# GoatWu/AdaLog

Hardware: AMD Instinct MI355X
Metric: calib_images_per_sec (higher is better)
Workload: dtype bf16

## Files before the change

### adalog_amd/_lib.py

```python
import ctypes as C
import os

_HERE = os.path.dirname(os.path.abspath(__file__))
LIB_PATH = os.environ.get("ADALOG_LIB") or os.path.join(_HERE, "csrc", "libadalog_hip.so")

p, i32, i64, f32, f64 = C.c_void_p, C.c_int, C.c_int64, C.c_float, C.c_double

ABI_VERSION = 2

SIGNATURES = {
    "adalog_abi_version": (i32, []),
    "adalog_last_error": (C.c_char_p, []),
    "adalog_last_kernel": (C.c_char_p, []),
    "adalog_uniform_fake_quant_f32": (i32, [p, p, p, i64, p, p, i64, i64, i32, i32, p]),
    "adalog_pack_uniform": (i32, [p, i64, i64, i64, i64, i64, i64, p, p, i64, i64, i64, i64, i64, i32, i32, p, i64, p, i32, p]),
    "adalog_pack_raw_f32": (i32, [p, i64, i64, i64, i64, i64, i64, p, i64, p]),
    "adalog_pack_split3_bf16": (i32, [p, i64, i64, i64, i64, i64, i64, p, i64, p]),
    "adalog_gemm_score": (i32, [i32, p, p, i64, i64, i64, i64, i32, i32, i64, i64, i32, i32, i32, p, i64, i64, i64, i32,
                                p, i64, i64, f32, p, i64, i64, i64, p, i64, i64, i64, p, p, p, i64, p, i64, i64, i64, i32, i32, p]),
    "adalog_gemm_score_layout": (i64, [i32, i32, i32, i32, i32, i32, i32, i32, i64, i64, i32, p, p, p]),
    "adalog_log2_shift": (i32, [p, p, i64, f32, p]),
    "adalog_score_act_fused_ok": (i32, [i32, i64, i32, i64, i32, i32]),
    "adalog_score_act_fused_workspace_bytes": (i64, [i64, i64]),
    "adalog_score_act_fused": (i32, [p, i32, i64, p, p, i64, i32, p, p, p, p, p, i32, i32, p, f32, i32, f32, f64, p, i64, p, p]),
# ... 65 lines not shown
    "adalog_select_hist": (i32, [p, i64, i64, i32, i32, i32, i64, i32, i32, i32, p, p]),
    "adalog_select_pick": (i32, [p, i64, i32, i32, p, i32, p]),
    "adalog_select_quantile_out": (i32, [p, i64, i32, p, i32, p, p]),
    "adalog_select_value_out": (i32, [p, i64, i32, p, p]),
    "adalog_uniform_int_f32": (i32, [p, p, i64, p, p, i32, p]),
    "adalog_permute_heads": (i32, [p, p, i64, i64, i32, i32, i32, i32, p]),
    "adalog_merge_heads": (i32, [p, p, p, p, p, i64, i64, i32, i32, i32, p]),
    "adalog_qkv_quant_chunks": (i32, [i64, i64, i32]),
    "adalog_qkv_split_quant": (i32, [p, p, p, p, i64, i64, i32, i32, p, p, p, p, p]),
    "adalog_qkv_merge_quant_backward": (i32, [p, p, p, p, p, i64, i64, i32, i32, p, p, p, p, p, p, p]),
    "adalog_scaled_softmax": (i32, [p, p, i64, i32, f32, p]),
    "adalog_scaled_softmax_backward": (i32, [p, p, p, i64, i32, f32, p]),
    "adalog_uniform_fq_backward_blocks": (i32, [i64, i64, i64]),
    "adalog_uniform_fq_backward": (i32, [p, p, p, i64, p, p, i64, i64, i32, i32, p, p, p, p]),
    "adalog_uniform_fake_quant_drop_f32": (i32, [p, p, i64, p, p, i64, i64, i32, i32, f32, p, i32, p]),
    "adalog_uniform_fq_backward_drop": (i32, [p, p, p, i64, p, p, i64, i64, i32, i32, p, p, p, f32, p, i32, p]),
    "adalog_log_fake_quant_drop_f32": (i32, [p, p, i64, p, p, i32, p, i32, i32, f32, p, i32, p]),
    "adalog_log_fq_backward_drop": (i32, [p, p, p, i64, p, p, i32, p, i32, p, p, i32, f32, p, i32, p]),
    "adalog_qkv_split_quant_drop": (i32, [p, p, p, p, i64, i64, i32, i32, p, p, p, p, p, p, p, p]),
    "adalog_qkv_merge_quant_backward_drop": (i32, [p, p, p, p, p, i64, i64, i32, i32, p, p, p, p, p, p, p, p, p, p]),
    "adalog_adaround": (i32, [p, p, p, p, i64, i64, p, p, i32, i32, i32, p]),
    "adalog_adaround_t": (i32, [p, p, p, p, i64, i64, p, p, i32, i32, p]),
    "adalog_alpha_step_multi": (i32, [p, p, p, p, p, p, p, p, p, p, i32, f32, p, f32, f32, f32, p, f32, p, f32, p, p, p]),
    "adalog_round_loss": (i32, [p, i64, f32, p, p, p, f32, p, i32, p, p]),
    "adalog_round_loss_multi_workspace": (i64, [p, i32]),
    "adalog_round_loss_multi": (i32, [p, p, p, i32, f32, p, f32, p, p, p, p]),
    "adalog_gemm_win_ok": (i32, [i32, i32, i32, i32, i32, i32, i64]),
    "adalog_gemm_score_gen": (i32, [i32, p, i64, i32, i32, i64, i64, i32, i32, p, i64, i64, p, i32, p, i64, i32, p, i64, i64, f32, p, i64,
                              i64, p, i64, p]),
    "adalog_gemm_score_gen_ok": (i32, [i32, i32, i32, i32, i32, i32, i64, i64]),
    "adalog_gemm_score_avq": (i32, [p, i64, i32, i32, i64, i64, i32, i32, p, i64, i64, p, p, i32, p, i64, i32, p, i64, i64, f32, p, i64, i64,
                              p, i64, p]),
    "adalog_gemm_score_avq_ok": (i32, [i32, i32, i32, i32, i32, i64, i64, i32]),
    "adalog_gemm_mixed_ok": (i32, [i32, i32, i32, i32, i32, i64]),
    "adalog_gemm_mixed_ktrim": (i32, [i32, i32, i32, i32, i32, i64]),
    "adalog_rec_loss": (i32, [p, p, i64, f32, p, p, p]),
    "adalog_rec_loss_backward": (i32, [p, p, i64, f32, p, p, p]),
    "adalog_brecq_init": (i32, []),
    "adalog_adam_multi": (i32, [p, p, p, p, p, i32, f32, p, f32, f32, f32, p, p]),
    "adalog_gemm_f32x3_workspace_bytes": (i64, [i32, i32, i32, i32, i32, i32, i32, i32, i32]),
    "adalog_gemm_f32x3_planes_workspace_bytes": (i64, [i32, i32, i32, i32, i32, i32]),
    "adalog_gemm_f32x3_planes": (i32, [p, i64, p, i64, p, i64, i32, i32, i32, i32, i64, i64, p, f32, p, i32, i32, p, p]),
    "adalog_gemm_f32x3": (i32, [p, i64, i32, p, i64, i32, p, i64, i32, i32, i32, i32, i64, i64, i64, p, f32, p, i32, i32, i32, p, p]),
    "adalog_gemm_f32x3_add": (i32, [p, i64, i32, p, i64, i32, p, i64, i32, i32, i32, i32, i64, i64, i64, p, f32, p, i32, i32, i32, p, p, p]),
    "adalog_gemm_f32x3_g2": (i32, [p, i64, i32, p, i64, i32, p, i64, i32, i32, i32, i32, i64, i64, i64, i32, i64, i64, i64, p, f32, p,
                             i32, i32, i32, p, p]),
    "adalog_shift_fold": (i32, [p, p, p, p, i32, i32, p, p]),
    "adalog_minmax_rows": (i32, [p, i32, i32, i32, p, p, p]),
    "adalog_absminmax_cols": (i32, [p, i64, i32, i32, p, p, p]),
    "adalog_packed_row_words": (i64, [i64, i32]),
    "adalog_pack_codes_f32": (i32, [p, i64, i64, i64, p, p, i32, i32, p, p]),
    "adalog_unpack_codes": (i32, [p, i64, i64, p, p, i32, i32, i32, p, i64, p]),
    "adalog_err_stats_workspace_bytes": (i64, [i64, i64, i64]),
    "adalog_err_stats_f32": (i32, [p, p, i64, i64, i64, p, p, i64, p]),
    "adalog_mean_err_workspace_bytes": (i64, [i64, i64, i64]),
    "adalog_mean_err_f32": (i32, [p, p, i64, i64, i64, p, p, i64, p]),
    "adalog_uniform_code_hist_f32": (i32, [p, i64, p, p, i64, i64, i32, p, p]),
    "adalog_log_code_hist_f32": (i32, [p, i64, p, p, i32, p, i32, p, p]),
    "adalog_gptq_sweep_ok": (i32, [i64, i64]),
    "adalog_gptq_sweep_f32": (i32, [p, i64, i64, i64, p, p, i32, i32, p, i64, p, p, p, p]),
    "adalog_bit_cost_ok": (i32, [i64, i64, i32]),
    "adalog_bit_cost_workspace_bytes": (i64, [i64, i64, i32]),
    "adalog_bit_cost_f32": (i32, [p, i64, i64, i64, p, p, i32, p, i32, p, i64, p, p, i64, p]),
}

class FpcsTail(C.Structure):
# ... 41 lines not shown
```

### adalog_amd/csrc/gemm_score.hip

```cpp
#include "common.h"
#include "fpcs_tail.h"
#include <stdlib.h>

#pragma clang fp contract(fast)

namespace {

#include "gemm_types.inc"
#include "gemm_k_basic.inc"
#include "gemm_k_stream.inc"
#include "gemm_k_slab.inc"
#include "gemm_k_grp.inc"
#include "gemm_finish.inc"

}

static int device_cus() {
    static int n_cu = 0;
    if (!n_cu) {
        int dev = 0; hipDeviceProp_t prop;
        if (hipGetDevice(&dev) == hipSuccess && hipGetDeviceProperties(&prop, dev) == hipSuccess) n_cu = prop.multiProcessorCount;
        if (n_cu <= 0) n_cu = 256;
    }
    return n_cu;
}

static int pick_tm_out(int M, int64_t col_tiles_x_groups) {
    if (const char* e = getenv("ADALOG_GEMM_TM")) { const int v = atoi(e); if (v == 1 || v == 2 || v == 4) return v; }
    const int64_t want = 2 * (int64_t)device_cus();
    const int tms[3] = {4, 2, 1};
    for (int i = 0; i < 3; ++i)
        if ((int64_t)cdiv(M, 64 * tms[i]) * col_tiles_x_groups >= want) return tms[i];
    return 1;
}

static int pick_tm(int M, bool scoring) {
    if (const char* e = getenv("ADALOG_GEMM_TM")) {
        const int v = atoi(e);
        if (v == 1 || v == 2 || (v == 4 && !scoring)) return v;
    }
    double best = 0.0;
    int tms[3] = {scoring ? 2 : 4, 2, 1};
    double util[3];
    for (int i = 0; i < 3; ++i) {
        const int bm = 64 * tms[i];
// ... 603 lines not shown
extern "C" int adalog_gemm_score_avq(const void* A, int64_t sAg, int M, int N, int64_t Kp, int64_t k_valid, int G, int gmod,
                                     const float* x, int64_t ldx, int64_t sg, const float* q, const uint32_t* lut, int n_bits,
                                     const float* ref, int64_t sRg, int P, const float* sa, int64_t sa_c, int64_t sa_g, float sa_mul,
                                     const float* sb, int64_t sb_c, int64_t sb_g, float* partial, int64_t partial_elems,
                                     void* stream) {
    ADALOG_ARG_CHECK(A && x && q && lut && ref && sa && sb && partial, "gemm_score_avq: null pointer");
    ADALOG_ARG_CHECK(avq_ok(M, N, G, gmod, P, k_valid, Kp, n_bits), "gemm_score_avq: shape not taken (adalog_gemm_score_avq_ok)");
    ADALOG_ARG_CHECK((((uintptr_t)A) & 15) == 0 && (((uintptr_t)partial) & 7) == 0, "gemm_score_avq: operand / accumulator alignment");
    const Layout L = layout_of(M, N * P, 1, G, gmod, P, 1, true, k_valid * 2, Kp * 2, true, 1);
    ADALOG_ARG_CHECK(partial_elems >= L.elems, "gemm_score_avq: partial buffer too small");
    GemmArgs p{};
    p.A = (const uint8_t*)A; p.sAg = sAg * 2; p.M = M; p.N = N * P; p.Kb = Kp * 2; p.Kvb = k_valid * 2; p.C = 1; p.G = G; p.gmod = gmod;
    p.ref = ref; p.ldr = 1; p.sRg = sRg; p.ref_cs = M; p.ref_div = P;
    p.sa = sa; p.sa_c = sa_c; p.sa_g = sa_g; p.sa_mul = sa_mul; p.sb = sb; p.sb_c = sb_c; p.sb_g = sb_g;
    p.wg_acc = (double*)partial; p.partial = partial;
    p.gen_x = x; p.gen_ldx = ldx; p.gen_sg = sg; p.gen_K = (int)k_valid; p.gen_q = q; p.gen_lut = lut; p.gen_nb = 1 << n_bits;
    wave_chunks(p, N, L.wgs, G, cdiv(N, AVQ_ROWS));
    const int nks = k_valid <= 64 ? 4 : 13;
    const size_t lut_b = (((size_t)(p.gen_nb + 1) * P + 3) & ~(size_t)3) * 4;
    const size_t rows_b = (size_t)4 * ((size_t)AVQ_ROWS * (nks * 16 + 64) + 4 * 64 * 2) * 4;
    const size_t acc_b = (size_t)gmod * 256 * 8;
    const size_t shm = lut_b + rows_b > acc_b ? lut_b + rows_b : acc_b;
    hipStream_t st = (hipStream_t)stream;
    const unsigned wgs = (unsigned)L.wgs;
    const int e = nks == 13 ? (M > 32 ? adalog_launch<k_gemm_avq<4, 13, 2>>("k_gemm_avq<13,bf16>", 80 * 1024, wgs, 256, shm, st, p)
                                      : adalog_launch<k_gemm_avq<4, 13, 1>>("k_gemm_avq<13,bf16>", 80 * 1024, wgs, 256, shm, st, p))
                            : (M > 32 ? adalog_launch<k_gemm_avq<4, 4, 2>>("k_gemm_avq<4,bf16>", 80 * 1024, wgs, 256, shm, st, p)
                                      : adalog_launch<k_gemm_avq<4, 4, 1>>("k_gemm_avq<4,bf16>", 80 * 1024, wgs, 256, shm, st, p));
    if (e) return e;
    ADALOG_LAUNCH_CHECK("adalog_gemm_score_avq");
    return 0;
}

extern "C" int adalog_gemm_score_gen_ok(int dtype, int M, int N, int G, int gmod, int ref_div, int64_t k_valid, int64_t Kp) {
    if (!(dtype == 0 || dtype == 3) || k_valid < 16 || k_valid > 64 || k_valid % 16 || ref_div < 1 || N % ref_div != 0 || G % gmod) return 0;
    const MmCall c = shape_call(dtype, M, N, G, gmod, ref_div, k_valid, Kp, 1);
    const Route r = route_of(c, call_layout(c, true));
    return (r == R_WIN || r == R_GRPW) ? 1 : 0;
}

static Layout gen_layout(int dtype, int M, int64_t T, int K, int64_t Kp, int P) {
    Layout L{};
    if (!(dtype == 0 || dtype == 3) || !(P == 64 || P == 128 || P == 256) || T < 1 || T * P >= ((int64_t)1 << 31) || K < 16 || K % 16 != 0 ||
        Kp < K) return L;
    return layout_of(M, (int)(T * P), 1, 1, 1, P, 1, true, (int64_t)K, Kp, true, dtype, true);
}

extern "C" int adalog_score_act_gen_ok(int dtype, int M, int64_t T, int K, int64_t Kp, int P) {
    static const int use_gen = getenv("ADALOG_SLAB_GEN") ? atoi(getenv("ADALOG_SLAB_GEN")) : 1;
    if (!use_gen || Kp % BK3 != 0) return 0;
    const Layout L = gen_layout(dtype, M, T, K, Kp, P);
    return (L.slab && L.acc) ? 1 : 0;
}

extern "C" int adalog_score_act_gen_wgs(int dtype, int M, int64_t T, int K, int64_t Kp, int P) {
    const Layout L = gen_layout(dtype, M, T, K, Kp, P);
    return (L.slab && L.acc) ? L.wgs : -1;
}

extern "C" int64_t adalog_score_act_gen_workspace_bytes(int dtype, int M, int64_t T, int K, int64_t Kp, int P) {
    const Layout L = gen_layout(dtype, M, T, K, Kp, P);
    if (!(L.slab && L.acc)) return -1;
    return L.elems * (int64_t)sizeof(float) + ((int64_t)M * 4 + 15) / 16 * 16;
}

extern "C" int adalog_score_act_gen(int dtype, const void* Wp, int M, int64_t Kp, const float* x, int64_t T, int K, int64_t ldx,
// ... 180 lines not shown
```

### adalog_amd/ops.py

```python
from __future__ import annotations

import ctypes
import math
import os
from typing import Optional, Tuple

import torch

from . import _lib, _torch_ops

I8, BF16, F32, FP8 = 0, 1, 2, 3
BF16_FP8 = 4
GEMM_EVENTS = None
_ESZ = {I8: 1, BF16: 2, F32: 4, FP8: 1}
_TORCH_DT = {I8: torch.int8, BF16: torch.bfloat16, F32: torch.float32, FP8: torch.float8_e4m3fn}


def _stream():
    return torch.cuda.current_stream().cuda_stream


def _top(name, *args):
    try:
        return getattr(torch.ops.adalog, name)(*args)
# ... 608 lines not shown


def gemm_score_avq_ok(M: int, N: int, G: int, gmod: int, P: int, k_valid: int, Kp: int, n_bits: int) -> bool:
    return bool(_lib.load().adalog_gemm_score_avq_ok(int(M), int(N), int(G), int(gmod), int(P), int(k_valid), int(Kp), int(n_bits)))


def gemm_score_avq(A, src3, q_all, lut, n_bits: int, M: int, N: int, P: int, G: int, gmod: int, ref, sa: Strided, sb: Strided,
                   norm: float, sa_mul: float = 1.0):
    lib = _lib.load()
    sa, sb = sa.checked(), sb.checked()
    src3, q_all, ref = _f32c(src3, "src"), _f32c(q_all, "q"), _f32c(ref, "ref")
    Gs, Ns, K = src3.shape
    Kp = A.shape[-1]
    assert (Gs, Ns) == (G, N) and A.shape[-2] == M and A.is_contiguous() and A.dtype == torch.bfloat16
    assert lut.dtype == torch.int32 and lut.is_contiguous() and lut.shape == ((1 << n_bits) + 1, P)
    assert ref.shape[-1] == M and ref.shape[-2] == N
    sAg = 0 if A.shape[1] == 1 and G > 1 else A.stride(1)
    sRg = 0 if G == 1 else M * N
    n_part, MT, Npad, mode = _layout(M, N * P, 1, G, gmod, P, 1, BF16, Kp, K, True)
    partial = torch.empty((n_part + 1) // 2, dtype=torch.float64, device=A.device).view(torch.float32)
    if GEMM_EVENTS is not None:
        ev0, ev1 = torch.cuda.Event(enable_timing=True), torch.cuda.Event(enable_timing=True)
        ev0.record()
    rc = lib.adalog_gemm_score_avq(A.data_ptr(), sAg, M, N, Kp, K, G, gmod, src3.data_ptr(), K, N * K, q_all.data_ptr(), lut.data_ptr(),
                                   int(n_bits), ref.data_ptr(), sRg, P, sa.t.data_ptr(), sa.c, sa.g, float(sa_mul), sb.t.data_ptr(),
                                   sb.c, sb.g, partial.data_ptr(), n_part, _stream())
    if GEMM_EVENTS is not None:
        ev1.record()
        GEMM_EVENTS.append((BF16, M, N, K, P, G, ev0, ev1, lib.adalog_last_kernel().decode()))
    _lib.check(rc, "adalog_gemm_score_avq")
    return PendingScores(partial, MT, Npad if mode != 1 else N, Npad, P, G, gmod, False, False, mode, norm, N).finish()


def gemm_out(dtype: int, A, B, M: int, N: int, G: int, gmod: int, sa: Strided, sb: Strided, bias: Optional[Strided],
             sa_mul: float = 1.0, addend=None, heads_last: int = 0):
    lib = _lib.load()
    sa, sb = sa.checked(), sb.checked()
    bias = None if bias is None else bias.checked()
    Kp = A.shape[-1]
    assert B.shape[-1] == Kp and A.dtype == _TORCH_DT[dtype] and B.dtype == _TORCH_DT[dtype]
    sAg = 0 if A.shape[1] == 1 and G > 1 else A.stride(1)
    sBg = 0 if B.shape[1] == 1 and G > 1 else B.stride(1)
    if addend is not None or heads_last:
        assert dtype in (I8, BF16) and sa.c == 0 and sb.c == 0 and (bias is None or bias.c == 0)
        H = int(heads_last)
        if H:
            assert G % H == 0 and addend is None
            out = torch.empty((G // H, M, H, N), dtype=torch.float32, device=A.device)
            ldo, sOg, gi, sOo = H * N, N, H, M * H * N
        else:
            addend = _f32c(addend, "addend")
            assert addend.numel() == G * M * N
            out = torch.empty((G, M, N), dtype=torch.float32, device=A.device)
            ldo, sOg, gi, sOo = N, M * N, 0, 0
        rc = lib.adalog_gemm_out_ex(dtype, A.data_ptr(), B.data_ptr(), sAg, sBg, M, N, Kp, G, gmod, sa.t.data_ptr(), sa.g, float(sa_mul),
                                    sb.t.data_ptr(), sb.g, sb.n, None if bias is None else bias.t.data_ptr(),
                                    0 if bias is None else bias.g, 0 if bias is None else bias.n, _ptr(addend), out.data_ptr(),
                                    ldo, sOg, gi, sOo, _stream())
        _lib.check(rc, "adalog_gemm_out_ex")
        return out
    out = torch.empty((G, M, N), dtype=torch.float32, device=A.device)
    rc = lib.adalog_gemm_score(dtype, A.data_ptr(), B.data_ptr(), 0, sAg, 0, sBg, M, N, Kp, 0, 1, G, gmod, None, 0, 0, 1, 1,
                               sa.t.data_ptr(), sa.c, sa.g, float(sa_mul), sb.t.data_ptr(), sb.c, sb.g, sb.n,
                               None if bias is None else bias.t.data_ptr(),
                               0 if bias is None else bias.c, 0 if bias is None else bias.g,
                               0 if bias is None else bias.n, None, None,
# ... 1278 lines not shown
```

### adalog_amd/quant_layers/matmul.py

```python
import os

import torch
import torch.nn as nn

from .. import backend, search, train_mm
from ..ops import BF16, BF16_FP8, FP8, I8, Strided, pad_k
from ..ops import mixed_k_align as ops_mixed_k_align
from ..quantizers.logarithm import AdaLogQuantizer
from ..quantizers.uniform import UniformQuantizer

MAX_PACK_BYTES = int(os.environ.get('ADALOG_MAX_PACK_GIB', '8')) << 30
GEN_MM = os.environ.get('ADALOG_GEN_MM', 'all')
GEN_AVQ = os.environ.get('ADALOG_GEN_AVQ', '1') != '0'
MIXED_B_SEARCH = os.environ.get('ADALOG_MIXED_B', '1') != '0'
AV_KTRIM = os.environ.get('ADALOG_AV_KTRIM', '1') != '0'


class MinMaxQuantMatMul(nn.Module):
    def __init__(self, A_bit=8, B_bit=8, mode="raw"):
        super().__init__()
        self.mode = mode
        self.A_quantizer = UniformQuantizer(n_bits=A_bit, symmetric=True, channel_wise=False)
        self.B_quantizer = UniformQuantizer(n_bits=B_bit, symmetric=True, channel_wise=False)
        self.raw_input = None
        self.raw_out = None
        self.tmp_input = None
        self.tmp_out = None
        self.calibrated = False

    def forward(self, A, B, a_pre=False, b_pre=False):
        if self.mode == 'raw':
            return A @ B
        if self.mode == "quant_forward":
            return self.quant_forward(A, B, a_pre, b_pre)
        raise NotImplementedError

    def quant_input_A(self, x):
        return self.A_quantizer(x)

    def quant_input_B(self, x):
        return self.B_quantizer(x)

    def quant_forward(self, A, B, a_pre=False, b_pre=False):
        assert self.calibrated, f"Module should be calibrated before run quant_forward for {self}"
        a_sim = A if a_pre else self.quant_input_A(A)
        b_sim = B if b_pre else self.quant_input_B(B)
        if a_sim.requires_grad or b_sim.requires_grad:
            return train_mm.matmul(a_sim, b_sim, heads_last=getattr(self, 'out_heads_last', False))
# ... 90 lines not shown

    def _kalign(self, dt=None):
        G, S, K, Sp = self._dims()
        if self.eq_n not in (64, 128, 256):
            return 128
        if dt in (I8, FP8) and K <= 32 and self._cand_chunk(G * max(S, Sp) * 32) >= self.eq_n:
            be, H = backend.get(), self._heads()
            if be.gemm_win_ok(dt, Sp, S, G, H, self.eq_n, K) and be.gemm_win_ok(dt, S, Sp, G, H, self.eq_n, K):
                return 32
        esz = 1 if dt in (I8, FP8) else 2
        whole = self._cand_chunk(G * max(S, Sp) * pad_k(K, BF16 if esz == 2 else I8, 64) * esz) >= self.eq_n
        return 64 if whole else 128

    def _mixed_kalign(self):
        be = backend.get()
        G, S, K, Sp = self._dims()
        kp = 0
        if AV_KTRIM and K > 64 and hasattr(be, "gemm_mixed_ktrim"):
            kp = be.gemm_mixed_ktrim(S, Sp, G, self._heads(), self.eq_n, K)
        return ops_mixed_k_align(K, kp)

    def _pack_fixed(self, which, dt=I8):
        be = backend.get()
        H = self._heads()
        A, B = self.raw_input
        al = self._kalign(dt)
        if which == "A":
            s, z = self._q_params(self.A_quantizer)
            return be.pack_uniform(self._a3(A), s, z, 1, 0, H, 1 if H > 1 else 0, 0, self.A_quantizer.n_bits, dt, k_align=al)
        s, z = self._q_params(self.B_quantizer)
        return be.pack_uniform(self._bt3_packable(B), s, z, 1, 0, H, 1 if H > 1 else 0, 0, self.B_quantizer.n_bits, dt,
                               k_align=al)

    def _score(self, which, fixed, scale, zp, dt=I8, fixed_sa=None, sa_mul=1.0, defer=False):
        be = backend.get()
        H = self._heads()
        G, S, K, Sp = self._dims()
        A, B = self.raw_input
        P = scale.shape[0]
        src = self._a3(A) if which == "A" else self._bt3_packable(B)
        bits = self.A_quantizer.n_bits if which == "A" else self.B_quantizer.n_bits
        rows = S if which == "A" else Sp
        mixed = dt == BF16_FP8
        cdt = FP8 if mixed else dt
        esz = 2 if dt == BF16 else 1
        al = ops_mixed_k_align(K, fixed.shape[-1])[0] if mixed else self._kalign(dt)
        chunk = self._cand_chunk(G * rows * pad_k(K, cdt, al) * esz)
        if mixed and chunk < P:
            raise RuntimeError("the mixed softmax.v search scores all candidates in one launch")
        pg = 1 if H > 1 else 0
        mrows, ncols = (Sp, S) if which == "A" else (S, Sp)
        if (GEN_MM != '0' and dt in (I8, FP8) and chunk >= P and K % 16 == 0 and K <= 64 and hasattr(be, "gemm_score_gen")
                and (dt != FP8 or bits <= 4) and src.dtype == torch.float32
                and be.gemm_score_gen_ok(dt, mrows, ncols, G, H, P, K, fixed.shape[-1])
                and (GEN_MM == 'all' or be.gemm_win_ok(dt, mrows, ncols, G, H, P, K))):
            sc, zc = scale.contiguous(), zp.contiguous()
            sb = Strided(sc, c=H, g=pg)
            if which == "A":
                sa, ref = Strided(self.B_quantizer.scale.data.view(-1), g=pg), self._ref3()
            else:
                sa = fixed_sa if fixed_sa is not None else Strided(self.A_quantizer.scale.data.view(-1), g=pg)
                ref = self._ref3_t()
            pend = be.gemm_score_gen(dt, fixed, src, zc, bits, mrows, ncols, P, G, H, ref, sa, sb, self.head_channel_wise,
                                     self._norm(A, S, Sp), sa_mul=sa_mul)
            return pend if defer else pend.finish()
        out = []
        for s0 in range(0, P, chunk):
            e = min(P, s0 + chunk)
            sc, zc = scale[s0:e].contiguous(), zp[s0:e].contiguous()
            cand = be.pack_uniform(src, sc, zc, e - s0, H, H, pg, 0, bits, cdt, c_inner=True, k_align=al)
            sb = Strided(sc, c=H, g=pg)
            if which == "A":
                sa = Strided(self.B_quantizer.scale.data.view(-1), g=pg)
                out.append(be.gemm_score(dt, fixed, cand, Sp, S, e - s0, G, H, self._ref3(), sa, sb, None,
                                         self.head_channel_wise, False, self._norm(A, S, Sp), sa_mul=sa_mul,
                                         ref_div=e - s0, order=2, ref_transposed=True, defer=defer and chunk >= P))
            else:
                sa = fixed_sa if fixed_sa is not None else Strided(self.A_quantizer.scale.data.view(-1), g=pg)
                out.append(be.gemm_score(dt, fixed, cand, S, Sp, e - s0, G, H, self._ref3_t(), sa, sb, None,
                                         self.head_channel_wise, False, self._norm(A, S, Sp), sa_mul=sa_mul,
                                         ref_div=e - s0, order=2, ref_transposed=True, defer=defer and chunk >= P))
        return out[0] if len(out) == 1 else torch.cat(out, 0)

    def _commit(self, quantizer, scale, zp):
        search.commit_param(quantizer.scale, scale)
        search.commit_param(quantizer.zero_point, zp)
        quantizer.forget_codes_fit()

    def packed_codes_fit(self):
        b_ok = self.B_quantizer.codes_fit(-256, 256) if isinstance(self, PostSoftmaxAsymmetricallyBatchingQuantMatMul) \
            else self.B_quantizer.codes_fit(-128, 127)
        return b_ok and (isinstance(self, PostSoftmaxAsymmetricallyBatchingQuantMatMul) or self.A_quantizer.codes_fit(-128, 127))

    def _fpcs(self, which, fpcs_width=16, steps=6, fixed=None, dt=I8, fixed_sa=None, sa_mul=1.0, checked=False):
        if not checked and search.round_is_redundant(self, which, self.B_quantizer if which == "A" else self.A_quantizer):
            return
        x = self.raw_input[0] if which == "A" else self.raw_input[1]
        scale, zp, delta = search.matmul_grid(x, self.B_quantizer.n_bits, self.eq_n, self.head_channel_wise)
        if fixed is None:
            fixed = self._pack_fixed("B" if which == "A" else "A", dt)
        fn = lambda s, z, t: self._score(which, fixed, s, z, dt, fixed_sa, sa_mul, defer=True)
        q = self.A_quantizer if which == "A" else self.B_quantizer
        res = search.fpcs(scale, zp, None, delta, fn, steps, fpcs_width, self.eq_n, None,
                          commit_to=search.commit_targets(q.scale, q.zero_point, None))
        if res is not None:
            self._commit(q, res[0], res[1])

    def _init_from_grid(self, which):
        x = self.raw_input[0] if which == "A" else self.raw_input[1]
        scale, zp, _ = search.matmul_grid(x, self.B_quantizer.n_bits, self.eq_n, self.head_channel_wise)
        q = self.A_quantizer if which == "A" else self.B_quantizer
        self._commit(q, scale[-2], zp[-2])
        q.inited = True

    def hyperparameter_searching(self):
        search.forget_grids()
        if not self.fpcs:
            raise NotImplementedError("non-FPCS search is not part of the accelerated path")
        self._initialize_calib_parameters()
        search.begin_rounds(self)
        self._init_from_grid("A")
        self._init_from_grid("B")
        G, S, K, Sp = self._dims()
        dt = search.int_operand_dtype(self.A_quantizer.n_bits, self.B_quantizer.n_bits,
                                      self._cand_chunk(G * max(S, Sp) * pad_k(K, I8)), prefer_fp8=K <= 64)
        for _ in range(self.search_round):
            self._fpcs("A", steps=self.steps, dt=dt)
            self._fpcs("B", steps=self.steps, dt=dt)
        self.calibrated = True
        search.begin_rounds(self)
        search.forget_grids()
        del self.raw_input, self.raw_out
        self._ref_t = self._ref_t_key = None
        self._bt_c = self._bt_key = None
# ... 91 lines not shown
        return bool(be.gemm_mixed_ok(S, Sp, G, self._heads(), self.eq_n, K))

    def _search_best_A_log_base(self):
        be = backend.get()
        aq = self.A_quantizer
        if search.round_is_redundant(self, "Aq", self.B_quantizer):
            return
        q_all, scores = self._score_A_log_base()
        idx = search.argbest(scores, 1)
        best_q = be.fpcs_next(q_all.view(-1, 1), None, None, idx, 1, 0, None, None, None)[0]
        aq.q.data.copy_(best_q.view(aq.q.shape).to(aq.q.dtype))
        self._q_host = int(aq.q.item())
        aq.update_table(self._q_host)

    def hyperparameter_searching(self):
        search.forget_grids()
        if not self.fpcs:
            raise NotImplementedError("non-FPCS search is not part of the accelerated path")
        self._initialize_calib_parameters()
        search.begin_rounds(self)
        self._init_from_grid("B")
        A = self.raw_input[0]
        dev = A.device
        for _ in range(self.search_round):
            self._search_best_A_log_base()
            if search.round_is_redundant(self, "B", self.A_quantizer):
                continue
            mixed = self._mixed_B_search()
            qv = search.const_tensor([float(self._q_host)], dev)
            K = A.shape[-1]
            ap = self._pack_A_adalog(self._a3(A), qv, self.A_quantizer.scale.data.view(-1), 1, True,
                                     k_align=self._mixed_kalign()[1] if mixed else self._kalign())
            self._fpcs("B", steps=self.steps, fixed=ap, dt=BF16_FP8 if mixed else BF16,
                       fixed_sa=Strided(self.A_quantizer.scale.data.view(-1)), sa_mul=self._ts32(), checked=True)
        self.calibrated = True
        search.begin_rounds(self)
        search.forget_grids()
        del self.raw_input, self.raw_out
        self._ref_t = self._ref_t_key = None
        self._bt_c = self._bt_key = None
        return None

    def quant_forward(self, A, B, a_pre=False, b_pre=False):
        assert self.calibrated, f"Module should be calibrated before run quant_forward for {self}"
        if a_pre or b_pre or self._training() or self.A_quantizer.training_mode or not self.packed_codes_fit():
            return MinMaxQuantMatMul.quant_forward(self, A, B, a_pre, b_pre)
        be = backend.get()
        H = self._heads()
        pg = 1 if H > 1 else 0
        lead = A.shape[:-2]
        S, Sp = A.shape[-2], B.shape[-1]
        if self._q_host is None:
            self._q_host = int(self.A_quantizer.q.item())
        qv = search.const_tensor([float(self._q_host)], A.device)
        a3, bt3 = self._a3(A), self._bt3(B)
        ap = self._pack_A_adalog(a3, qv, self.A_quantizer.scale.data.view(-1), 1, True)
        sB, zB = self._q_params(self.B_quantizer)
        bp = be.pack_uniform(bt3, sB, zB, 1, 0, H, pg, 0, self.B_quantizer.n_bits, BF16)
        out = be.gemm_out(BF16, ap, bp, S, Sp, a3.shape[0], H, Strided(self.A_quantizer.scale.data.view(-1)),
                          Strided(sB, g=pg), None, sa_mul=self._ts32())
        return out.view(*lead, S, Sp)

    def _load_from_state_dict(self, *a, **k):
        super()._load_from_state_dict(*a, **k)
        self._q_host = None
```

### include/adalog_hip.h

```cpp
#ifndef ADALOG_HIP_H
#define ADALOG_HIP_H
#include <stdint.h>
#ifdef __cplusplus
extern "C" {
#endif

#define ADALOG_ABI_VERSION 2
int adalog_abi_version(void);
const char* adalog_last_error(void);
const char* adalog_last_kernel(void);

int adalog_uniform_fake_quant_f32(const float* x, float* y, uint8_t* bins, int64_t n, const float* scale,
                                  const float* zero_point, int64_t n_channels, int64_t inner, int n_bits, int symmetric,
                                  void* stream);

int adalog_log_fake_quant_f32(const float* x, float* y, uint8_t* bins, int64_t n, const float* scale, const int64_t* q,
                              const float* table1, const float* table2, int n_bits, const float* shift, int sub_shift,
                              int train_form, int pre, void* stream);

int adalog_pack_uniform(const float* x, int64_t G, int64_t R, int64_t K, int64_t sxg, int64_t sxr, int64_t sxk,
                        const float* scale, const float* zero_point, int64_t C, int64_t pc, int64_t gmod, int64_t pg,
                        int64_t pr, int n_bits, int out_dtype, void* out, int64_t Kp, int32_t* rowsum, int c_inner,
                        void* stream);
int adalog_pack_adalog_bf16(const float* x, int64_t G, int64_t R, int64_t K, int64_t sxg, int64_t sxr, int64_t sxk,
                            const float* scale, const float* qv, int64_t C, int64_t pc, int64_t gmod, int64_t pg,
                            int n_bits, const float* mant37, const float* shift, int clamp_u, void* out, int64_t Kp,
                            int c_inner, int pre, void* stream);
int adalog_pack_raw_f32(const float* x, int64_t G, int64_t R, int64_t K, int64_t sxg, int64_t sxr, int64_t sxk, void* out,
                        int64_t Kp, void* stream);
int adalog_pack_split3_bf16(const float* x, int64_t G, int64_t R, int64_t K, int64_t sxg, int64_t sxr, int64_t sxk, void* out,
                            int64_t Kt, void* stream);

int adalog_gemm_mixed_ok(int M, int N, int G, int gmod, int ref_div, int64_t k_valid);
int adalog_gemm_mixed_ktrim(int M, int N, int G, int gmod, int ref_div, int64_t k_valid);
int adalog_gemm_score(int dtype, const void* A, const void* B, int64_t sAc, int64_t sAg, int64_t sBc, int64_t sBg, int M,
                      int N, int64_t Kp, int64_t k_valid, int C, int G, int gmod, const float* ref, int64_t ldr, int64_t sRg, int64_t ref_cs,
                      int ref_div, const float* sa, int64_t sa_c, int64_t sa_g, float sa_mul, const float* sb, int64_t sb_c,
                      int64_t sb_g, int64_t sb_n, const float* bias, int64_t bi_c, int64_t bi_g, int64_t bi_n,
                      const float* row_scale, const float* row_bias, float* partial, int64_t partial_elems, float* out,
                      int64_t ldo, int64_t sOc, int64_t sOg, int order, int reduce_cols, void* stream);
int64_t adalog_gemm_score_layout(int M, int N, int C, int G, int gmod, int ref_div, int reduce_cols, int dtype, int64_t Kp,
                                 int64_t k_valid, int ref_transposed, int* MT, int* Npad, int* mode);

int adalog_gemm_win_ok(int dtype, int M, int N, int G, int gmod, int ref_div, int64_t k_valid);
int adalog_gemm_score_gen(int dtype, const void* A, int64_t sAg, int M, int N, int64_t Kp, int64_t k_valid, int G, int gmod,
                          const float* x, int64_t ldx, int64_t sg, const float* zp, int n_bits, const float* ref, int64_t sRg,
                          int ref_div, const float* sa, int64_t sa_c, int64_t sa_g, float sa_mul, const float* sb, int64_t sb_c,
                          int64_t sb_g, float* partial, int64_t partial_elems, void* stream);
int adalog_gemm_score_gen_ok(int dtype, int M, int N, int G, int gmod, int ref_div, int64_t k_valid, int64_t Kp);
int adalog_gemm_score_avq(const void* A, int64_t sAg, int M, int N, int64_t Kp, int64_t k_valid, int G, int gmod, const float* x,
                          int64_t ldx, int64_t sg, const float* q, const uint32_t* lut, int n_bits, const float* ref, int64_t sRg,
                          int P, const float* sa, int64_t sa_c, int64_t sa_g, float sa_mul, const float* sb, int64_t sb_c,
                          int64_t sb_g, float* partial, int64_t partial_elems, void* stream);
int adalog_gemm_score_avq_ok(int M, int N, int G, int gmod, int P, int64_t k_valid, int64_t Kp, int n_bits);
int adalog_finish_scores(const float* partial, float* scores, int MT, int N, int Npad, int C, int G, int gmod, int keep_h,
                         int keep_n, int cand_inner, double norm, void* workspace, int64_t workspace_bytes, void* stream);
int64_t adalog_finish_workspace_bytes(int MT, int N, int C, int G, int keep_n, int cand_inner);
int adalog_finish_topk_next(const float* partial, float* scores, int MT, int N, int Npad, int C, int G, int gmod, int keep_h,
                            int keep_n, int cand_inner, double norm, void* workspace, int64_t workspace_bytes, int k,
                            const float* scale, const float* zp, const float* third, int new_cnt, const float* lin, float* delta,
                            int has_clamp, float clamp_min, float* out_scale, float* out_zp, float* out_third, void* stream);

int adalog_log2_shift(const float* x, float* out, int64_t n, float shift, void* stream);
int adalog_score_act_fused_ok(int M, int64_t T, int K, int64_t Kp, int P, int n_bits);
int64_t adalog_score_act_fused_workspace_bytes(int64_t T, int64_t Kp);
int adalog_score_act_fused(const void* Wp, int M, int64_t Kp, const float* x, const float* Lx, int64_t T, int K,
                           const float* ref, const float* row_scale, const float* row_bias, const float* scale,
                           const float* qv, int P, int n_bits, const float* mant37, float shift, int clamp_u, float sa_mul,
                           double norm, void* workspace, int64_t workspace_bytes, float* scores, void* stream);

int adalog_topk(const float* scores, int P, int cols, int k, int* idx, void* stream);
typedef struct adalog_fpcs_tail {
    int32_t k, new_cnt, has_clamp;
    float clamp_min;
    const float* scale; const float* zp; const float* third;
    const float* lin;
    const float* delta_in; float* delta_out;
    float* out_scale; float* out_zp; float* out_third;
} adalog_fpcs_tail;
int adalog_topk_next_tail(const float* scores, int P, int cols, const adalog_fpcs_tail* tail, int* idx_out, void* stream);
int adalog_finish_topk_next_tail(const float* partial, float* scores, int MT, int N, int Npad, int C, int G, int gmod, int keep_h,
                                 int keep_n, int cand_inner, double norm, void* workspace, int64_t workspace_bytes,
                                 const adalog_fpcs_tail* tail, void* stream);
int adalog_topk_next(const float* scores, int P, int cols, int k, const float* scale, const float* zp, const float* third,
                     int new_cnt, const float* lin, float* delta, int has_clamp, float clamp_min, float* out_scale,
                     float* out_zp, float* out_third, int* idx_out, void* stream);
int adalog_fpcs_next(const float* scale, const float* zp, const float* third, int cols, const int* idx, int k, int new_cnt,
// ... 237 lines not shown
```

Measured before the change: 37.64.

## Add fused on-the-fly B quantization kernel for attn·V candidate scoring with K>64

New measurement: 38.84 (median of 6 runs). 3.2% higher.

```diff
diff --git a/adalog_amd/_lib.py b/adalog_amd/_lib.py
--- a/adalog_amd/_lib.py
+++ b/adalog_amd/_lib.py
@@ -121,6 +121,9 @@
     "adalog_gemm_score_avq": (i32, [p, i64, i32, i32, i64, i64, i32, i32, p, i64, i64, p, p, i32, p, i64, i32, p, i64, i64, f32, p, i64, i64,
                               p, i64, p]),
     "adalog_gemm_score_avq_ok": (i32, [i32, i32, i32, i32, i32, i64, i64, i32]),
+    "adalog_gemm_score_avw": (i32, [p, i64, i32, i32, i64, i64, i32, i32, p, i64, i64, p, i32, p, i64, i32, p, i64, i64, f32, p, i64, i64,
+                              p, i64, p]),
+    "adalog_gemm_score_avw_ok": (i32, [i32, i32, i32, i32, i32, i64, i64, i32]),
     "adalog_gemm_mixed_ok": (i32, [i32, i32, i32, i32, i32, i64]),
     "adalog_gemm_mixed_ktrim": (i32, [i32, i32, i32, i32, i32, i64]),
     "adalog_rec_loss": (i32, [p, p, i64, f32, p, p, p]),
diff --git a/adalog_amd/csrc/gemm_k_avw.inc b/adalog_amd/csrc/gemm_k_avw.inc
--- /dev/null
+++ b/adalog_amd/csrc/gemm_k_avw.inc
@@ -0,0 +1,165 @@
+struct AvwCand { float s, inv, lo, hi; };
+__device__ __forceinline__ uint4 avw_gen8(const v4u& xa, const v4u& xb, const AvwCand& c) {
+#pragma clang fp contract(off)
+    const float x[8] = {__uint_as_float(xa.x), __uint_as_float(xa.y), __uint_as_float(xa.z), __uint_as_float(xa.w),
+                        __uint_as_float(xb.x), __uint_as_float(xb.y), __uint_as_float(xb.z), __uint_as_float(xb.w)};
+    float k[8], dm = 0.0f;
+#pragma unroll
+    for (int e = 0; e < 8; ++e) {
+        const float t = x[e] * c.inv;
+        k[e] = rintf(t);
+        dm = fmaxf(dm, fabsf(t - k[e]));
+    }
+    if (__builtin_expect(dm > 0.4999f, 0)) {
+#pragma unroll
+        for (int e = 0; e < 8; ++e) k[e] = rintf(x[e] / c.s);
+    }
+    uint32_t w[4];
+#pragma unroll
+    for (int e = 0; e < 4; ++e) {
+        const uint32_t v0 = __float_as_uint(__builtin_amdgcn_fmed3f(k[2 * e], c.lo, c.hi));
+        const uint32_t v1 = __float_as_uint(__builtin_amdgcn_fmed3f(k[2 * e + 1], c.lo, c.hi));
+        w[e] = __builtin_amdgcn_perm(v1, v0, 0x07060302u);
+    }
+    return make_uint4(w[0], w[1], w[2], w[3]);
+}
+
+template <int NJ, bool R7>
+__global__ __launch_bounds__(NJ * 64, 2) void k_gemm_avw_gen(GemmArgs p) {
+#if defined(__HIP_DEVICE_COMPILE__)
+    constexpr int NKS = 13, ASL = 25, ARB = ASL * 16, NT = NJ * 64, LA = 2;
+    extern __shared__ __attribute__((aligned(16))) uint8_t lds[];
+    const int tid = threadIdx.x, lane = tid & 63;
+    const int w = __builtin_amdgcn_readfirstlane(tid >> 6);
+    const int frow = lane & 31, fkg = lane >> 5;
+    const int M = p.M, KbA = (int)p.KbA;
+    const int nrb = R7 ? 7 : (M + 31) >> 5;
+    const int NB = p.N >> 5;
+    const int CB = p.slab_R, NCH = p.slab_U;
+    const int items = p.G * NCH;
+    const int ci = w * 32 + frow;
+    double* wacc = p.wg_acc + (int64_t)blockIdx.x * p.gmod * 256;
+    for (int i = tid; i < p.gmod * 256; i += NT) wacc[i] = 0.0;
+
+    const int base0 = frow * ARB + fkg * 32, base6 = min(192 + frow, M) * ARB + fkg * 32;
+    auto aoff = [&](int rb) { return R7 ? (rb < 6 ? base0 + rb * 32 * ARB : base6) : min(rb * 32 + frow, M) * ARB + fkg * 32; };
+    const int xvoff = fkg * 64;
+
+    for (int item = blockIdx.x; item < items; item += gridDim.x) {
+        const int g = item / NCH, c = item - g * NCH, gh = g % p.gmod;
+        const int blk0 = c * CB, nblk = min(CB, NB - blk0);
+        const int d0 = blk0 / NJ, nd = nblk / NJ;
+        __syncthreads();
+        {
+            const uint8_t* ag = p.A + (int64_t)g * p.sAg;
+            const int nsl = min(ASL, KbA >> 4);
+            for (int idx = tid; idx < (M + 1) * ASL + 4; idx += NT) {
+                const int r = idx / ASL, s = idx - r * ASL;
+                uint4 v = make_uint4(0, 0, 0, 0);
+                if (r < M && s < nsl) v = *reinterpret_cast<const uint4*>(ag + (int64_t)r * KbA + s * 16);
+                *reinterpret_cast<uint4*>(lds + r * ARB + s * 16) = v;
+            }
+        }
+        __syncthreads();
+
+        AvwCand cand;
+        {
+            const int64_t pi = ci * p.sb_c + gh * p.sb_g;
+            const float z = rintf(p.gen_zp[pi]);
+            cand.s = p.sb[pi]; cand.inv = __builtin_amdgcn_rcpf(cand.s); cand.lo = -z; cand.hi = p.gen_qmax - z;
+        }
+        const float nal = -(p.sa[ci * p.sa_c + gh * p.sa_g] * p.sa_mul * p.sb[ci * p.sb_c + gh * p.sb_g]);
+        const int64_t xbytes = ((int64_t)(p.N / (NJ * 32)) * p.gen_ldx) * 4;
+        const __amdgpu_buffer_rsrc_t rx = __builtin_amdgcn_make_buffer_rsrc((void*)(p.gen_x + (int64_t)g * p.gen_sg), 0,
+                                                                            (int)min(xbytes, (int64_t)0x7ffffffe), 0x00020000);
+        const float* refg = p.ref + (int64_t)g * p.sRg;
+        auto load_x = [&](int d, int i, v4u& xa, v4u& xb) {
+            const int so = d * (int)p.gen_ldx * 4;
+            xa = __builtin_amdgcn_raw_buffer_load_b128(rx, xvoff + (32 * (i >> 1) + 8 * (i & 1)) * 4, so, 0);
+            xb = __builtin_amdgcn_raw_buffer_load_b128(rx, xvoff + (32 * (i >> 1) + 8 * (i & 1)) * 4 + 16, so, 0);
+        };
+        auto load_a = [&](int i, uint4 (&af)[7]) {
+#pragma unroll
+            for (int rb = 0; rb < 7; ++rb)
+                if (R7 || rb < nrb) af[rb] = *reinterpret_cast<const uint4*>(lds + aoff(rb) + (i >> 1) * 64 + (i & 1) * 16);
+        };
+        auto load_ref = [&](int d, int rb, float (&r)[16]) {
+            const float* rp = refg + (int64_t)d * p.ref_cs;
+#pragma unroll
+            for (int q = 0; q < 4; ++q) {
+                const int rr = rb * 32 + 8 * q + 4 * fkg;
+                if (rr + 4 <= M) {
+#pragma unroll
+                    for (int e = 0; e < 4; ++e) r[4 * q + e] = rp[rr + e];
+                } else {
+#pragma unroll
+                    for (int e = 0; e < 4; ++e) r[4 * q + e] = rr + e < M ? rp[rr + e] : 0.0f;
+                }
+            }
+        };
+
+        v2f csr[7];
+#pragma unroll
+        for (int rb = 0; rb < 7; ++rb) csr[rb] = (v2f){0.0f, 0.0f};
+
+        v4u xq[NKS + LA][2];
+#pragma unroll
+        for (int i = 0; i < LA; ++i) load_x(d0, i, xq[i][0], xq[i][1]);
+        for (int dd = 0; dd < nd; ++dd) {
+            const int d = d0 + dd, dn = d0 + min(dd + 1, nd - 1);
+            v16f acc[7];
+#pragma unroll
+            for (int rb = 0; rb < 7; ++rb)
+#pragma unroll
+                for (int e = 0; e < 16; ++e) acc[rb][e] = 0.0f;
+            uint4 bq = avw_gen8(xq[0][0], xq[0][1], cand);
+#pragma unroll
+            for (int i = 0; i < NKS; ++i) {
+                uint4 af[7];
+                load_a(i, af);
+                if (i + LA < NKS) load_x(d, i + LA, xq[i + LA][0], xq[i + LA][1]);
+                else load_x(dn, i + LA - NKS, xq[i + LA][0], xq[i + LA][1]);
+                uint4 bn = bq;
+                if (i + 1 < NKS) bn = avw_gen8(xq[i + 1][0], xq[i + 1][1], cand);
+                if (i + 1 == 12 && fkg) bn = make_uint4(0, 0, 0, 0);
+#pragma unroll
+                for (int rb = 0; rb < 7; ++rb)
+                    if (R7 || rb < nrb) mma<1>(af[rb], bq, acc[rb]);
+                bq = bn;
+                __builtin_amdgcn_sched_barrier(0);
+            }
+#pragma unroll
+            for (int i = 0; i < LA; ++i) { xq[i][0] = xq[NKS + i][0]; xq[i][1] = xq[NKS + i][1]; }
+            float rc[16], rn[16];
+            load_ref(d, 0, rc);
+#pragma unroll
+            for (int rb = 0; rb < 7; ++rb) {
+                if (R7 || rb < nrb) {
+                    if (rb + 1 < 7 && (R7 || rb + 1 < nrb)) load_ref(d, rb + 1, rn);
+#pragma unroll
+                    for (int q = 0; q < 4; ++q) {
+                        const float e0 = __builtin_fmaf(acc[rb][q * 4 + 0], nal, rc[q * 4 + 0]);
+                        const float e1 = __builtin_fmaf(acc[rb][q * 4 + 1], nal, rc[q * 4 + 1]);
+                        const float e2 = __builtin_fmaf(acc[rb][q * 4 + 2], nal, rc[q * 4 + 2]);
+                        const float e3 = __builtin_fmaf(acc[rb][q * 4 + 3], nal, rc[q * 4 + 3]);
+                        csr[rb].x = __builtin_fmaf(e0, e0, csr[rb].x); csr[rb].y = __builtin_fmaf(e1, e1, csr[rb].y);
+                        csr[rb].x = __builtin_fmaf(e2, e2, csr[rb].x); csr[rb].y = __builtin_fmaf(e3, e3, csr[rb].y);
+                    }
+#pragma unroll
+                    for (int e = 0; e < 16; ++e) rc[e] = rn[e];
+                }
+            }
+        }
+        double v = 0.0;
+#pragma unroll
+        for (int rb = 0; rb < 7; ++rb) {
+            if (R7 || rb < nrb) {
+                float cs = csr[rb].x + csr[rb].y;
+                cs += __shfl_xor(cs, 32);
+                v += (double)cs;
+            }
+        }
+        if (fkg == 0) wacc[gh * 256 + ci] += v;
+    }
+#endif
+}
diff --git a/adalog_amd/csrc/gemm_score.hip b/adalog_amd/csrc/gemm_score.hip
--- a/adalog_amd/csrc/gemm_score.hip
+++ b/adalog_amd/csrc/gemm_score.hip
@@ -11,6 +11,7 @@
 #include "gemm_k_stream.inc"
 #include "gemm_k_slab.inc"
 #include "gemm_k_grp.inc"
+#include "gemm_k_avw.inc"
 #include "gemm_finish.inc"
 
 }
@@ -680,6 +681,45 @@
     return 0;
 }
 
+static int avw_wgs(int M, int N, int G, int gmod, int P, int64_t k_valid, int64_t Kp, int n_bits) {
+    if (!(P == 64 || P == 128 || P == 256) || M < 1 || M > 224 || N < 32 || N % 32 || k_valid < 1 || k_valid > 200 || Kp < k_valid || Kp % 8 ||
+        n_bits < 1 || n_bits > 4 || gmod < 1 || G < 1 || G % gmod || (int64_t)N * P >= ((int64_t)1 << 30))
+        return 0;
+    const Layout L = layout_of(M, N * P, 1, G, gmod, P, 1, true, k_valid * 2, Kp * 2, true, 1);
+    return (L.stream && L.acc && !L.slab && L.wgs >= 1) ? L.wgs : 0;
+}
+extern "C" int adalog_gemm_score_avw_ok(int M, int N, int G, int gmod, int P, int64_t k_valid, int64_t Kp, int n_bits) {
+    return avw_wgs(M, N, G, gmod, P, k_valid, Kp, n_bits);
+}
+extern "C" int adalog_gemm_score_avw(const void* A, int64_t sAg, int M, int N, int64_t Kp, int64_t k_valid, int G, int gmod,
+                                     const float* x, int64_t ldx, int64_t sg, const float* zp, int n_bits, const float* ref, int64_t sRg,
+                                     int P, const float* sa, int64_t sa_c, int64_t sa_g, float sa_mul, const float* sb, int64_t sb_c,
+                                     int64_t sb_g, float* partial, int64_t partial_elems, void* stream) {
+    ADALOG_ARG_CHECK(A && x && zp && ref && sa && sb && partial, "gemm_score_avw: null pointer");
+    const int wgs = avw_wgs(M, N, G, gmod, P, k_valid, Kp, n_bits);
+    ADALOG_ARG_CHECK(wgs > 0, "gemm_score_avw: shape not taken (adalog_gemm_score_avw_ok)");
+    ADALOG_ARG_CHECK((((uintptr_t)A) & 15) == 0 && (sAg * 2) % 16 == 0 && (((uintptr_t)partial) & 7) == 0 && (((uintptr_t)x) & 3) == 0,
+                     "gemm_score_avw: operand / accumulator alignment");
+    ADALOG_ARG_CHECK(ldx >= k_valid && (int64_t)N * ldx * 4 < ((int64_t)1 << 31), "gemm_score_avw: rows of x shorter than K, or a group of x beyond 32-bit addressing");
+    ADALOG_ARG_CHECK(partial_elems >= (int64_t)2 * wgs * gmod * BN2, "gemm_score_avw: partial buffer too small");
+    GemmArgs p{};
+    p.A = (const uint8_t*)A; p.sAg = sAg * 2; p.M = M; p.N = N * P; p.Kb = Kp; p.KbA = Kp * 2; p.Kvb = k_valid; p.C = 1; p.G = G; p.gmod = gmod;
+    p.ref = ref; p.ldr = 1; p.sRg = sRg; p.ref_cs = M; p.ref_div = P;
+    p.sa = sa; p.sa_c = sa_c; p.sa_g = sa_g; p.sa_mul = sa_mul; p.sb = sb; p.sb_c = sb_c; p.sb_g = sb_g;
+    p.wg_acc = (double*)partial; p.partial = partial;
+    p.gen_x = x; p.gen_ldx = ldx; p.gen_sg = sg; p.gen_K = (int)k_valid; p.gen_zp = zp; p.gen_qmax = (float)((1 << n_bits) - 1);
+    grp_chunks(p, N * P, wgs, G);
+    const size_t shm = (size_t)(M + 1) * 400 + 64;
+    hipStream_t st = (hipStream_t)stream;
+    if (const int e = with_nj(P, [&](auto nj) {
+            constexpr int NJ = decltype(nj)::value;
+            return M > 192 ? adalog_launch<k_gemm_avw_gen<NJ, true>>("k_gemm_avw_gen<13,bf16>", 160 * 1024, (unsigned)wgs, NJ * 64, shm, st, p)
+                           : adalog_launch<k_gemm_avw_gen<NJ, false>>("k_gemm_avw_gen<13,bf16>", 160 * 1024, (unsigned)wgs, NJ * 64, shm, st, p);
+        })) return e;
+    ADALOG_LAUNCH_CHECK("adalog_gemm_score_avw");
+    return 0;
+}
+
 extern "C" int adalog_gemm_score_gen_ok(int dtype, int M, int N, int G, int gmod, int ref_div, int64_t k_valid, int64_t Kp) {
     if (!(dtype == 0 || dtype == 3) || k_valid < 16 || k_valid > 64 || k_valid % 16 || ref_div < 1 || N % ref_div != 0 || G % gmod) return 0;
     const MmCall c = shape_call(dtype, M, N, G, gmod, ref_div, k_valid, Kp, 1);
diff --git a/adalog_amd/ops.py b/adalog_amd/ops.py
--- a/adalog_amd/ops.py
+++ b/adalog_amd/ops.py
@@ -664,6 +664,39 @@
     return PendingScores(partial, MT, Npad if mode != 1 else N, Npad, P, G, gmod, False, False, mode, norm, N).finish()
 
 
+def gemm_score_avw_ok(M: int, N: int, G: int, gmod: int, P: int, k_valid: int, Kp: int, n_bits: int) -> int:
+    return int(_lib.load().adalog_gemm_score_avw_ok(int(M), int(N), int(G), int(gmod), int(P), int(k_valid), int(Kp), int(n_bits)))
+
+
+def gemm_score_avw(A, src3, zp, n_bits: int, M: int, N: int, P: int, G: int, gmod: int, ref, sa: Strided, sb: Strided, keep_h: bool,
+                   norm: float, sa_mul: float = 1.0):
+    lib = _lib.load()
+    sa, sb = sa.checked(), sb.checked()
+    src3, zp, ref = _f32c(src3, "src"), _f32c(zp, "zero_point"), _f32c(ref, "ref")
+    Gs, Ns, K = src3.shape
+    Kp = A.shape[-1]
+    assert (Gs, Ns) == (G, N) and A.shape[-2] == M and A.is_contiguous() and A.dtype == torch.bfloat16 and zp.shape == sb.t.shape
+    assert ref.shape[-1] == M and ref.shape[-2] == N
+    wgs = gemm_score_avw_ok(M, N, G, gmod, P, K, Kp, n_bits)
+    if not wgs:
+        raise ValueError("gemm_score_avw: shape not taken (gemm_score_avw_ok)")
+    sAg = 0 if A.shape[1] == 1 and G > 1 else A.stride(1)
+    sRg = 0 if G == 1 else M * N
+    n_part = 2 * wgs * gmod * 256
+    partial = torch.empty(n_part // 2, dtype=torch.float64, device=A.device).view(torch.float32)
+    if GEMM_EVENTS is not None:
+        ev0, ev1 = torch.cuda.Event(enable_timing=True), torch.cuda.Event(enable_timing=True)
+        ev0.record()
+    rc = lib.adalog_gemm_score_avw(A.data_ptr(), sAg, M, N, Kp, K, G, gmod, src3.data_ptr(), K, N * K, zp.data_ptr(), int(n_bits),
+                                   ref.data_ptr(), sRg, P, sa.t.data_ptr(), sa.c, sa.g, float(sa_mul), sb.t.data_ptr(), sb.c, sb.g,
+                                   partial.data_ptr(), n_part, _stream())
+    if GEMM_EVENTS is not None:
+        ev1.record()
+        GEMM_EVENTS.append((BF16_FP8, M, N, K, P, G, ev0, ev1, lib.adalog_last_kernel().decode()))
+    _lib.check(rc, "adalog_gemm_score_avw")
+    return PendingScores(partial, wgs, 256, 256, P, G, gmod, keep_h, False, 2, norm, N)
+
+
 def gemm_out(dtype: int, A, B, M: int, N: int, G: int, gmod: int, sa: Strided, sb: Strided, bias: Optional[Strided],
              sa_mul: float = 1.0, addend=None, heads_last: int = 0):
     lib = _lib.load()
diff --git a/adalog_amd/quant_layers/matmul.py b/adalog_amd/quant_layers/matmul.py
--- a/adalog_amd/quant_layers/matmul.py
+++ b/adalog_amd/quant_layers/matmul.py
@@ -14,6 +14,7 @@
 GEN_AVQ = os.environ.get('ADALOG_GEN_AVQ', '1') != '0'
 MIXED_B_SEARCH = os.environ.get('ADALOG_MIXED_B', '1') != '0'
 AV_KTRIM = os.environ.get('ADALOG_AV_KTRIM', '1') != '0'
+AV_GEN = os.environ.get('ADALOG_AV_GEN', '1') != '0'
 
 
 class MinMaxQuantMatMul(nn.Module):
@@ -170,7 +171,7 @@
         return be.pack_uniform(self._bt3_packable(B), s, z, 1, 0, H, 1 if H > 1 else 0, 0, self.B_quantizer.n_bits, dt,
                                k_align=al)
 
-    def _score(self, which, fixed, scale, zp, dt=I8, fixed_sa=None, sa_mul=1.0, defer=False):
+    def _score(self, which, fixed, scale, zp, dt=I8, fixed_sa=None, sa_mul=1.0, defer=False, gen=False):
         be = backend.get()
         H = self._heads()
         G, S, K, Sp = self._dims()
@@ -202,6 +203,13 @@
             pend = be.gemm_score_gen(dt, fixed, src, zc, bits, mrows, ncols, P, G, H, ref, sa, sb, self.head_channel_wise,
                                      self._norm(A, S, Sp), sa_mul=sa_mul)
             return pend if defer else pend.finish()
+        if (gen and mixed and which == "B" and hasattr(be, "gemm_score_avw") and src.dtype == torch.float32 and src.is_contiguous()
+                and be.gemm_score_avw_ok(S, Sp, G, H, P, K, fixed.shape[-1], bits)):
+            sc, zc = scale.contiguous(), zp.contiguous()
+            sa = fixed_sa if fixed_sa is not None else Strided(self.A_quantizer.scale.data.view(-1), g=pg)
+            pend = be.gemm_score_avw(fixed, src, zc, bits, S, Sp, P, G, H, self._ref3_t(), sa, Strided(sc, c=H, g=pg),
+                                     self.head_channel_wise, self._norm(A, S, Sp), sa_mul=sa_mul)
+            return pend if defer else pend.finish()
         out = []
         for s0 in range(0, P, chunk):
             e = min(P, s0 + chunk)
@@ -230,14 +238,14 @@
             else self.B_quantizer.codes_fit(-128, 127)
         return b_ok and (isinstance(self, PostSoftmaxAsymmetricallyBatchingQuantMatMul) or self.A_quantizer.codes_fit(-128, 127))
 
-    def _fpcs(self, which, fpcs_width=16, steps=6, fixed=None, dt=I8, fixed_sa=None, sa_mul=1.0, checked=False):
+    def _fpcs(self, which, fpcs_width=16, steps=6, fixed=None, dt=I8, fixed_sa=None, sa_mul=1.0, checked=False, gen=False):
         if not checked and search.round_is_redundant(self, which, self.B_quantizer if which == "A" else self.A_quantizer):
             return
         x = self.raw_input[0] if which == "A" else self.raw_input[1]
         scale, zp, delta = search.matmul_grid(x, self.B_quantizer.n_bits, self.eq_n, self.head_channel_wise)
         if fixed is None:
             fixed = self._pack_fixed("B" if which == "A" else "A", dt)
-        fn = lambda s, z, t: self._score(which, fixed, s, z, dt, fixed_sa, sa_mul, defer=True)
+        fn = lambda s, z, t: self._score(which, fixed, s, z, dt, fixed_sa, sa_mul, defer=True, gen=gen)
         q = self.A_quantizer if which == "A" else self.B_quantizer
         res = search.fpcs(scale, zp, None, delta, fn, steps, fpcs_width, self.eq_n, None,
                           commit_to=search.commit_targets(q.scale, q.zero_point, None))
@@ -395,7 +403,8 @@
             ap = self._pack_A_adalog(self._a3(A), qv, self.A_quantizer.scale.data.view(-1), 1, True,
                                      k_align=self._mixed_kalign()[1] if mixed else self._kalign())
             self._fpcs("B", steps=self.steps, fixed=ap, dt=BF16_FP8 if mixed else BF16,
-                       fixed_sa=Strided(self.A_quantizer.scale.data.view(-1)), sa_mul=self._ts32(), checked=True)
+                       fixed_sa=Strided(self.A_quantizer.scale.data.view(-1)), sa_mul=self._ts32(), checked=True,
+                       gen=mixed and AV_GEN and K > 64)
         self.calibrated = True
         search.begin_rounds(self)
         search.forget_grids()
diff --git a/include/adalog_hip.h b/include/adalog_hip.h
--- a/include/adalog_hip.h
+++ b/include/adalog_hip.h
@@ -53,6 +53,11 @@
                           int P, const float* sa, int64_t sa_c, int64_t sa_g, float sa_mul, const float* sb, int64_t sb_c,
                           int64_t sb_g, float* partial, int64_t partial_elems, void* stream);
 int adalog_gemm_score_avq_ok(int M, int N, int G, int gmod, int P, int64_t k_valid, int64_t Kp, int n_bits);
+int adalog_gemm_score_avw(const void* A, int64_t sAg, int M, int N, int64_t Kp, int64_t k_valid, int G, int gmod, const float* x,
+                          int64_t ldx, int64_t sg, const float* zp, int n_bits, const float* ref, int64_t sRg, int P, const float* sa,
+                          int64_t sa_c, int64_t sa_g, float sa_mul, const float* sb, int64_t sb_c, int64_t sb_g, float* partial,
+                          int64_t partial_elems, void* stream);
+int adalog_gemm_score_avw_ok(int M, int N, int G, int gmod, int P, int64_t k_valid, int64_t Kp, int n_bits);
 int adalog_finish_scores(const float* partial, float* scores, int MT, int N, int Npad, int C, int G, int gmod, int keep_h,
                          int keep_n, int cand_inner, double norm, void* workspace, int64_t workspace_bytes, void* stream);
 int64_t adalog_finish_workspace_bytes(int MT, int N, int C, int G, int keep_n, int cand_inner);
```
